# mmbajo/PROBA-V

Measured on AMD Instinct MI355X. Metric: LR-patches/sec fwd+bwd (WDSR-B r12 t9, 16x16, bs128), higher is better.
Workload: dtype f32 (products as 3 scaled-fp16-piece MFMA products, f32 accumulate)

## Files before the change

proba-v_amd/csrc/kernels_direct.hip:

```cpp
#include "probav_common.h"
#include "x6_device.h"

namespace probav {

__device__ __forceinline__ int reflect_idx(int i, int n) {
    i = i < 0 ? -i : i;
    return i >= n ? 2 * n - 2 - i : i;
}

template <int COUT_T, int VEC>
__global__ __launch_bounds__(256) void conv_direct_fwd_kernel(
    ConvGeom g, const float* __restrict__ x, const float* __restrict__ gate, const float* __restrict__ w,
    const float* __restrict__ bias, const float* __restrict__ skip, float* __restrict__ y)
{
    const long nvox = (long)g.N * g.Ho * g.Wo * g.To;
    const long v = (long)blockIdx.x * 256 + threadIdx.x;
    if (v >= nvox) return;
    const int co0 = blockIdx.y * COUT_T;
    long r = v;
    const int t = (int)(r % g.To); r /= g.To;
    const int wo = (int)(r % g.Wo); r /= g.Wo;
    const int h = (int)(r % g.Ho);
    const int n = (int)(r / g.Ho);

// ... 103 lines not shown
#pragma unroll
            for (int dh = 0; dh < 3; ++dh)
#pragma unroll
                for (int dw = 0; dw < 3; ++dw)
#pragma unroll
                    for (int dt = 0; dt < 3; ++dt) {
                        const float xv = ip[(dh * Wp + dw) * Tp + dt];
                        const float4 q = wt[(dh * 3 + dw) * 3 + dt];
                        acc.x = fmaf(xv, q.x, acc.x); acc.y = fmaf(xv, q.y, acc.y); acc.z = fmaf(xv, q.z, acc.z); acc.w = fmaf(xv, q.w, acc.w);
                    }
            if (g.relu) { acc.x = fmaxf(acc.x, 0.f); acc.y = fmaxf(acc.y, 0.f); acc.z = fmaxf(acc.z, 0.f); acc.w = fmaxf(acc.w, 0.f); }
            *reinterpret_cast<float4*>(yrow + (long)v * 32 + 4 * cg) = acc;
            omax = fmaxf(fmaxf(omax, fmaxf(fabsf(acc.x), fabsf(acc.y))), fmaxf(fabsf(acc.z), fabsf(acc.w)));
        }
    }
    if (amax && n_prev >= 0) amax_commit(omax, amax + n_prev);
}

bool conv3d_cin1_forward_supported(const ConvGeom& g)
{
    return g.Cin == 1 && g.Cout == 32 && g.kh == 3 && g.kw == 3 && g.kt == 3 && g.ph == 1 && g.pw == 1 && g.pt == 1 && !g.reflect_hw && !g.reflect_t &&
           g.Ho == g.Hi && g.Wo == g.Wi && g.To == g.Ti && g.To >= 2 && (g.Wi + 2) * (g.Ti + 2) * 3 * sizeof(float) <= 48 * 1024;
}
int conv3d_cin1_forward(const ConvGeom& g, const float* x, const float* w, const float* bias, float* y, unsigned* amax, hipStream_t s)
{
    if (!conv3d_cin1_forward_supported(g)) { set_error("conv3d_cin1_forward: unsupported geometry", hipSuccess); return PROBAV_EINVAL; }
    const long nrows = (long)g.N * g.Ho;
    const size_t lds = (size_t)3 * (g.Wi + 2) * (g.Ti + 2) * sizeof(float);
    hipLaunchKernelGGL(conv3_cin1_fwd_kernel, dim3((unsigned)((nrows + C1_ROWS - 1) / C1_ROWS)), dim3(256), lds, s, g, x, w, bias, y, amax);
    return check_launch("conv3_cin1_fwd");
}

int conv3d_direct_forward(const ConvGeom& g, const float* x, const float* gate, const float* w,
                          const float* bias, const float* skip, float* y, hipStream_t s)
{
    if (g.N <= 0) return PROBAV_OK;
    if (g.Cout % 32 == 0) return launch_fwd<32>(g, x, gate, w, bias, skip, y, s);
    if (g.Cout % 25 == 0) return launch_fwd<25>(g, x, gate, w, bias, skip, y, s);
    if (g.Cout % 9 == 0)  return launch_fwd<9>(g, x, gate, w, bias, skip, y, s);
    if (g.Cout % 4 == 0)  return launch_fwd<4>(g, x, gate, w, bias, skip, y, s);
    return launch_fwd<1>(g, x, gate, w, bias, skip, y, s);
}

bool conv3d_up_forward_supported(const ConvGeom& g)
{
    return g.Cin == 32 && g.Cout == 9 && g.kh == 3 && g.kw == 3 && g.kt == 3 && g.ph == 0 && g.pw == 0 && g.pt == 0 && !g.reflect_hw && !g.reflect_t &&
           g.Ti == 3 && g.To == 1 && g.Ho == g.Hi - 2 && g.Wo == g.Wi - 2 && g.Wo == 16;
}
bool conv3d_up_bwd_data_supported(const ConvGeom& g)
{
    return g.Cin == 9 && g.Cout == 32 && g.kh == 3 && g.kw == 3 && g.kt == 3 && g.ph == 2 && g.pw == 2 && g.pt == 2 && !g.reflect_hw && !g.reflect_t &&
           g.Ti == 1 && g.To == 3 && g.Ho == g.Hi + 2 && g.Wo == g.Wi + 2 && g.Wi <= 30;
}
__global__ __launch_bounds__(256) void conv3_up_fwd_kernel(ConvGeom g, const float* __restrict__ x, const float* __restrict__ w,
                                                          const float* __restrict__ bias, float* __restrict__ y)
{
    extern __shared__ float up_lds[];
    float* sW = up_lds;
    float* sX = sW + 27 * 32 * 9;
    const int tid = threadIdx.x;
    const int rowf = g.Wi * 3 * 32;
    if ((reinterpret_cast<unsigned long>(w) & 15) == 0) {
        for (int i = tid; i < 27 * 32 * 9 / 4; i += 256) reinterpret_cast<float4*>(sW)[i] = reinterpret_cast<const float4*>(w)[i];
    } else {
        for (int i = tid; i < 27 * 32 * 9; i += 256) sW[i] = w[i];
    }
    const int wo = tid >> 4, kp = tid & 15;
    for (int row = blockIdx.x; row < g.N * g.Ho; row += gridDim.x) {
    const int n = row / g.Ho, h = row - n * g.Ho;
    __syncthreads();
    const float4* xr = reinterpret_cast<const float4*>(x + ((long)n * g.Hi + h) * rowf);
    for (int i = tid; i < 3 * rowf / 4; i += 256) reinterpret_cast<float4*>(sX)[i] = xr[i];
    __syncthreads();
    float acc[9];
#pragma unroll
    for (int j = 0; j < 9; ++j) acc[j] = 0.f;
#pragma unroll 2
    for (int q = 0; q < 54; ++q) {
        const int k = kp + 16 * q;
        const int tap = k >> 5, ci = k & 31;
        const int a = tap / 9, bc = tap - 9 * a, b = bc / 3, c = bc - 3 * b;
        const float xv = sX[a * rowf + ((wo + b) * 3 + c) * 32 + ci];
        const float* wr = sW + k * 9;
#pragma unroll
        for (int j = 0; j < 9; ++j) acc[j] = fmaf(xv, wr[j], acc[j]);
    }
#pragma unroll
    for (int j = 0; j < 9; ++j) {
        float v = acc[j];
#pragma unroll
        for (int m = 1; m < 16; m <<= 1) v += __shfl_xor(v, m, 64);
        acc[j] = v;
    }
    if (kp < 9) {
        float o = 0.f;
#pragma unroll
        for (int j = 0; j < 9; ++j) o = kp == j ? acc[j] : o;
        o += bias ? bias[kp] : 0.f;
        if (g.relu) o = fmaxf(o, 0.f);
        y[(((long)n * g.Ho + h) * g.Wo + wo) * 9 + kp] = o;
    }
    }
}
__global__ __launch_bounds__(256) void conv3_up_bwd_data_kernel(ConvGeom g, const float* __restrict__ dy, const float* __restrict__ wT,
                                                               const float* __restrict__ bias, float* __restrict__ dx, unsigned* __restrict__ amax)
{
    extern __shared__ float up_lds[];
    float* sW = up_lds;
    float* sD = sW + 27 * 9 * 32;
    const int tid = threadIdx.x;
    const int Wp = g.Wi + 4;
    if ((reinterpret_cast<unsigned long>(wT) & 15) == 0) {
        for (int i = tid; i < 27 * 9 * 32 / 4; i += 256) reinterpret_cast<float4*>(sW)[i] = reinterpret_cast<const float4*>(wT)[i];
    } else {
        for (int i = tid; i < 27 * 9 * 32; i += 256) sW[i] = wT[i];
    }
    __shared__ float red[4];
    for (int row = blockIdx.x; row < g.N * g.Ho; row += gridDim.x) {
    const int n = row / g.Ho, h = row - n * g.Ho;
    __syncthreads();
    for (int i = tid; i < 3 * Wp * 9; i += 256) {
        const int a = i / (Wp * 9), r = i - a * Wp * 9, wp = r / 9, co = r - 9 * wp;
        const int ih = h + a - 2, iw = wp - 2;
        sD[i] = (ih >= 0 && ih < g.Hi && iw >= 0 && iw < g.Wi) ? dy[(((long)n * g.Hi + ih) * g.Wi + iw) * 9 + co] : 0.f;
    }
    __syncthreads();
    float omax = 0.f;
    const int items = g.Wo * 3 * 8;
    for (int it = tid; it < items; it += 256) {
        const int cg = it & 7, wt = it >> 3, wo = wt / 3, t = wt - 3 * wo;
        float4 acc = bias ? make_float4(bias[4 * cg], bias[4 * cg + 1], bias[4 * cg + 2], bias[4 * cg + 3]) : make_float4(0.f, 0.f, 0.f, 0.f);
#pragma unroll
        for (int a = 0; a < 3; ++a)
#pragma unroll
            for (int b = 0; b < 3; ++b) {
                const float* dp = sD + (a * Wp + wo + b) * 9;
                const float* wp = sW + (((a * 3 + b) * 3 + (2 - t)) * 9) * 32 + 4 * cg;
#pragma unroll
                for (int co = 0; co < 9; ++co) {
                    const float d = dp[co];
                    const float4 q = *reinterpret_cast<const float4*>(wp + co * 32);
                    acc.x = fmaf(d, q.x, acc.x); acc.y = fmaf(d, q.y, acc.y); acc.z = fmaf(d, q.z, acc.z); acc.w = fmaf(d, q.w, acc.w);
                }
            }
        *reinterpret_cast<float4*>(dx + ((((long)n * g.Ho + h) * g.Wo + wo) * 3 + t) * 32 + 4 * cg) = acc;
        omax = fmaxf(fmaxf(omax, fmaxf(fabsf(acc.x), fabsf(acc.y))), fmaxf(fabsf(acc.z), fabsf(acc.w)));
    }
    if (amax) {
#pragma unroll
        for (int o = 32; o; o >>= 1) omax = fmaxf(omax, __shfl_xor(omax, o, 64));
        if ((tid & 63) == 0) red[tid >> 6] = omax;
        __syncthreads();
        if (tid == 0) {
            const float m = fmaxf(fmaxf(red[0], red[1]), fmaxf(red[2], red[3]));
            atomicMax(amax + n, __float_as_uint(m));
        }
    }
    }
}
int conv3d_up_forward(const ConvGeom& g, const float* x, const float* w, const float* bias, float* y, hipStream_t s)
{
    if (!conv3d_up_forward_supported(g)) { set_error("conv3d_up_forward: unsupported geometry", hipSuccess); return PROBAV_EINVAL; }
    const size_t lds = ((size_t)27 * 32 * 9 + (size_t)3 * g.Wi * 3 * 32) * sizeof(float);
    hipLaunchKernelGGL(conv3_up_fwd_kernel, dim3((unsigned)(g.N * g.Ho < 512 ? g.N * g.Ho : 512)), dim3(256), lds, s, g, x, w, bias, y);
    return check_launch("conv3_up_fwd");
}
int conv3d_up_bwd_data(const ConvGeom& g, const float* dy, const float* wT, const float* bias, float* dx, unsigned* amax, hipStream_t s)
{
    if (!conv3d_up_bwd_data_supported(g)) { set_error("conv3d_up_bwd_data: unsupported geometry", hipSuccess); return PROBAV_EINVAL; }
    const size_t lds = ((size_t)27 * 9 * 32 + (size_t)3 * (g.Wi + 4) * 9) * sizeof(float);
    hipLaunchKernelGGL(conv3_up_bwd_data_kernel, dim3((unsigned)(g.N * g.Ho < 768 ? g.N * g.Ho : 768)), dim3(256), lds, s, g, dy, wT, bias, dx, amax);
    return check_launch("conv3_up_bwd_data");
}

template <int KH, int KW, int KT, int CI_PER>
__global__ __launch_bounds__(256) void conv_direct_wgrad_kernel(
    ConvGeom g, const float* __restrict__ x, const float* __restrict__ dy, const float* __restrict__ gate,
    float* __restrict__ partial, float* __restrict__ partial_b, long vox_per_chunk)
{
    constexpr int TAPS = KH * KW * KT;
    const int tid = threadIdx.x;
    const int co = blockIdx.y * 32 + (tid & 31);
    const bool co_ok = co < g.Cout;
    const int ci0 = (blockIdx.z * 8 + (tid >> 5)) * CI_PER;
    const long nvox = (long)g.N * g.Ho * g.Wo * g.To;
    const long v0 = (long)blockIdx.x * vox_per_chunk;
    const long v1 = v0 + vox_per_chunk < nvox ? v0 + vox_per_chunk : nvox;

    float acc[TAPS][CI_PER];
#pragma unroll
    for (int tp = 0; tp < TAPS; ++tp)
#pragma unroll
        for (int k = 0; k < CI_PER; ++k) acc[tp][k] = 0.f;
    float accb = 0.f;
    const bool vec4 = (CI_PER % 4 == 0) && (g.Cin % 4 == 0) && (ci0 + CI_PER <= g.Cin);

    for (long v = v0; v < v1; ++v) {
        long r = v;
        const int t = (int)(r % g.To); r /= g.To;
        const int wo = (int)(r % g.Wo); r /= g.Wo;
        const int h = (int)(r % g.Ho);
        const int n = (int)(r / g.Ho);
        float d = 0.f;
        if (co_ok) {
            d = dy[v * g.Cout + co];
            if (gate) d = gate[v * g.Cout + co] > 0.f ? d : 0.f;
        }
        accb += d;
#pragma unroll
        for (int a = 0; a < KH; ++a) {
            int ih = h + a - g.ph;
            if (g.reflect_hw) ih = reflect_idx(ih, g.Hi);
            else if (ih < 0 || ih >= g.Hi) continue;
#pragma unroll
            for (int b = 0; b < KW; ++b) {
                int iw = wo + b - g.pw;
                if (g.reflect_hw) iw = reflect_idx(iw, g.Wi);
                else if (iw < 0 || iw >= g.Wi) continue;
// ... 415 lines not shown
```

proba-v_amd/csrc/kernels_small.hip:

```cpp
#include "probav_common.h"
#include "../../include/probav_hip.h"
#include <cstdlib>
#include <vector>
#include <functional>
#include <stdio.h>
#include <string.h>

namespace probav {

static thread_local char g_err[512] = "";
void set_error(const char* what, hipError_t e)
{
    if (e != hipSuccess) snprintf(g_err, sizeof(g_err), "%s: %s", what, hipGetErrorString(e));
    else snprintf(g_err, sizeof(g_err), "%s", what);
}
const char* last_error() { return g_err; }
int check_launch(const char* what)
{
    hipError_t e = hipGetLastError();
    if (e != hipSuccess) { set_error(what, e); return PROBAV_EHIP; }
    return PROBAV_OK;
}

__device__ __forceinline__ float wave_sum(float v)
// ... 233 lines not shown
        for (size_t i = (size_t)blockIdx.x * 256 + threadIdx.x; i < n; i += stride) m = fmaxf(m, fabsf(x[i]));
    }
#pragma unroll
    for (int o = 32; o; o >>= 1) m = fmaxf(m, __shfl_xor(m, o, 64));
    __shared__ float wm[4];
    if ((threadIdx.x & 63) == 0) wm[threadIdx.x >> 6] = m;
    __syncthreads();
    if (threadIdx.x == 0) {
        m = fmaxf(fmaxf(wm[0], wm[1]), fmaxf(wm[2], wm[3]));
        atomicMax(slot, __float_as_uint(m));
    }
}
int amax_tensor(const float* x, size_t per_sample, int N, unsigned* slots, hipStream_t s)
{
    if (N < 1) return PROBAV_OK;
    size_t blocks = (per_sample / 4 + 255) / 256;
    if (blocks < 1) blocks = 1;
    const size_t cap = N >= 2048 ? 1 : 2048 / (size_t)N;
    if (blocks > cap) blocks = cap;
    hipLaunchKernelGGL(amax_kernel, dim3((unsigned)blocks, (unsigned)N), dim3(256), 0, s, x, per_sample, slots);
    return check_launch("amax");
}

__global__ __launch_bounds__(256) void amax_columns_kernel(const float* __restrict__ w, long rows, int cols, unsigned* __restrict__ slots)
{
    __shared__ float part[256];
    const int per = 256 / cols, c = threadIdx.x % cols, r0 = threadIdx.x / cols;
    float m = 0.f;
    if (r0 < per) for (long r = r0; r < rows; r += per) m = fmaxf(m, fabsf(w[r * cols + c]));
    part[threadIdx.x] = m;
    __syncthreads();
    if (threadIdx.x < cols) {
        for (int k = 1; k < per; ++k) m = fmaxf(m, part[k * cols + threadIdx.x]);
        slots[threadIdx.x] = __float_as_uint(m);
    }
}
int amax_columns(const float* w, long rows, int cols, unsigned* slots, hipStream_t s)
{
    if (cols < 1 || cols > 256) { set_error("amax_columns: 1 <= cols <= 256", hipSuccess); return PROBAV_EINVAL; }
    hipLaunchKernelGGL(amax_columns_kernel, dim3(1), dim3(256), 0, s, w, rows, cols, slots);
    return check_launch("amax_columns");
}

__global__ __launch_bounds__(64) void wn_backward_kernel(const WnLayer* __restrict__ layers, int nl,
                                                        const float* __restrict__ params, const float* __restrict__ dweff,
                                                        const float* __restrict__ inv_norm, float* __restrict__ grads)
{
    int co;
    const WnLayer L = layers[find_layer(layers, nl, blockIdx.x, co)];
    const float* v = params + L.v_off;
    const float* dw = dweff + L.w_off;
    const int lane = threadIdx.x;
    float dot = 0.f;
    for (int k = lane; k < L.K; k += 64) dot = fmaf(dw[(long)k * L.Cout + co], v[(long)k * L.Cout + co], dot);
    dot = wave_sum(dot);
    const float inv = inv_norm[L.n_off + co];
    const float gg = params[L.g_off + co];
    const bool clamped = inv >= 1e6f;
    const float proj = clamped ? 0.f : dot * inv * inv;
    if (lane == 0) grads[L.g_off + co] = dot * inv;
    for (int k = lane; k < L.K; k += 64) {
        const long i = (long)k * L.Cout + co;
        grads[L.v_off + i] = gg * inv * (dw[i] - v[i] * proj);
    }
}

int wn_forward(const WnLayer* d_layers, int nlayers, int cout_total, int cin_total, const float* params,
               float* weff, float* weffT, float* inv_norm, unsigned* amax, hipStream_t s)
{
    hipLaunchKernelGGL(wn_forward_kernel<false>, dim3(cout_total), dim3(64), 0, s, d_layers, nlayers, const_cast<float*>(params), weff, weffT, inv_norm, amax,
                       (const float*)nullptr, (float*)nullptr, (float*)nullptr, OptCoef());
    int rc = check_launch("wn_forward");
    if (rc || !amax) return rc;
    hipLaunchKernelGGL(wn_rowmax_kernel, dim3(cin_total), dim3(64), 0, s, d_layers, nlayers, weff, amax + 2 * nlayers + cout_total, amax, params);
    return check_launch("wn_rowmax");
}
int optimizer_wn_step(const WnLayer* d_layers, int nlayers, int cout_total, int cin_total, float* params, const float* grad, float* m, float* v,
                      float lr, float b1, float b2, float eps, float c_g, float c_m, float c_v,
                      float* weff, float* weffT, float* inv_norm, unsigned* amax, hipStream_t s)
{
    OptCoef oc = {lr, b1, b2, eps, c_g, c_m, c_v};
    hipLaunchKernelGGL(wn_forward_kernel<true>, dim3(cout_total), dim3(64), 0, s, d_layers, nlayers, params, weff, weffT, inv_norm, amax, grad, m, v, oc);
    int rc = check_launch("optimizer_wn_step");
    if (rc || !amax) return rc;
    hipLaunchKernelGGL(wn_rowmax_kernel, dim3(cin_total), dim3(64), 0, s, d_layers, nlayers, weff, amax + 2 * nlayers + cout_total, amax, params);
    return check_launch("wn_rowmax");
}
int optimizer_wn_step_guarded(const WnLayer* d_layers, int nlayers, int cout_total, int cin_total, float* params, const float* grad, float* m, float* v,
                              float lr, float b1, float b2, float eps, float c_g, float c_m, float c_v,
                              float* weff, float* weffT, float* inv_norm, unsigned* amax, float* ema, float ema_mom, const probav_guard_ctl* ctl, hipStream_t s)
{
    OptCoef oc = {lr, b1, b2, eps, c_g, c_m, c_v};
    hipLaunchKernelGGL(wn_forward_guard_kernel, dim3(cout_total), dim3(64), 0, s, d_layers, nlayers, params, weff, weffT, inv_norm, amax, grad, m, v, oc, ctl, ema, ema_mom);
    int rc = check_launch("optimizer_wn_step_guarded");
    if (rc || !amax) return rc;
    hipLaunchKernelGGL(wn_rowmax_kernel, dim3(cin_total), dim3(64), 0, s, d_layers, nlayers, weff, amax + 2 * nlayers + cout_total, amax, params);
    return check_launch("wn_rowmax");
}
int wn_backward(const WnLayer* d_layers, int nlayers, int cout_total, const float* params,
                const float* dweff, const float* inv_norm, float* grads, hipStream_t s)
{
    hipLaunchKernelGGL(wn_backward_kernel, dim3(cout_total), dim3(64), 0, s, d_layers, nlayers, params, dweff, inv_norm, grads);
    return check_launch("wn_backward");
}

__global__ __launch_bounds__(256) void head_kernel(const float* __restrict__ x, float* __restrict__ xn,
                                                  float* __restrict__ mn, int nhw, int T, int C, float mean, float stdv, unsigned* __restrict__ zero, int nzero)
{
    const int i = blockIdx.x * 256 + threadIdx.x;
    for (int z = i; z < nzero; z += gridDim.x * 256) zero[z] = 0u;
    if (i >= nhw * C) return;
// ... 319 lines not shown

__device__ __forceinline__ int fold_srcs(int i, int n, int p, int (&u)[3])
{
    int c = 0;
    u[c++] = i + p;
    for (int j = 1; j <= p; ++j) {
        if (i == j) u[c++] = p - j;
        if (i == n - 1 - j) u[c++] = n - 1 + p + j;
    }
    return c;
}
__global__ __launch_bounds__(256) void reflect_fold3_kernel(const float* __restrict__ dpad, float* __restrict__ dx, int N, int H, int W,
                                                           int T, int C, int ph, int pw, int pt)
{
    const long i = (long)blockIdx.x * 256 + threadIdx.x;
    if (i >= (long)N * H * W * T * C) return;
    long r = i;
    const int c = (int)(r % C); r /= C;
    const int t = (int)(r % T); r /= T;
    const int w = (int)(r % W); r /= W;
    const int h = (int)(r % H);
    const int n = (int)(r / H);
    int hs[3], ws[3], ts[3];
    const int nh = fold_srcs(h, H, ph, hs), nw = fold_srcs(w, W, pw, ws), nt = fold_srcs(t, T, pt, ts);
    const int Hp = H + 2 * ph, Wp = W + 2 * pw, Tp = T + 2 * pt;
    float s = 0.f;
    for (int a = 0; a < nh; ++a)
        for (int b = 0; b < nw; ++b)
            for (int d = 0; d < nt; ++d)
                s += dpad[((((long)n * Hp + hs[a]) * Wp + ws[b]) * Tp + ts[d]) * C + c];
    dx[i] = s;
}
int reflect_fold3(const float* dpad, float* dx, int N, int H, int W, int T, int C, int ph, int pw, int pt, hipStream_t s)
{
    if (ph < 0 || pw < 0 || pt < 0 || ph > 2 || pw > 2 || pt > 2 || H <= 2 * ph || W <= 2 * pw || T <= 2 * pt) {
        set_error("reflect_fold3: pads must be 0..2 and smaller than half the extent", hipSuccess); return PROBAV_EINVAL;
    }
    const long n = (long)N * H * W * T * C;
    hipLaunchKernelGGL(reflect_fold3_kernel, dim3((unsigned)((n + 255) / 256)), dim3(256), 0, s, dpad, dx, N, H, W, T, C, ph, pw, pt);
    return check_launch("reflect_fold3");
}

__global__ __launch_bounds__(256) void clip_round_kernel(const float* __restrict__ in, float* __restrict__ out, size_t n, float lo, float hi)
{
    const size_t i = (size_t)blockIdx.x * 256 + threadIdx.x;
    if (i < n) out[i] = rintf(fminf(fmaxf(in[i], lo), hi));
}
int clip_round(const float* in, float* out, size_t n, float lo, float hi, hipStream_t s)
{
    hipLaunchKernelGGL(clip_round_kernel, dim3((unsigned)((n + 255) / 256)), dim3(256), 0, s, in, out, n, lo, hi);
    return check_launch("clip_round");
}

__global__ __launch_bounds__(256) void shift_loss_fwd_kernel(
    const float* __restrict__ hr, const uint8_t* __restrict__ mask, const float* __restrict__ pred, int S, int border,
    double* __restrict__ cand)
{
    const int b = blockIdx.x, i = blockIdx.y, lane = threadIdx.x & 63, wave = threadIdx.x >> 6;
    const int L = S - 2 * border, ns = 2 * border + 1, nshift = ns * ns;
    const float* H = hr + (long)b * S * S;
    const uint8_t* M = mask + (long)b * S * S;
    const float* P = pred + (long)b * S * S;
    for (int j = wave; j < ns; j += 4) {
        const int sft = i * ns + j;
        constexpr int U = 4;
        const int n = L * L;
        double cnt = 0.0, dsum = 0.0;
        for (int k0 = lane; k0 < n; k0 += 64 * U) {
            float m[U], h[U], q[U];
#pragma unroll
            for (int u = 0; u < U; ++u) {
                const int k = k0 + 64 * u < n ? k0 + 64 * u : k0;
                const int r = k / L, c = k - r * L;
                m[u] = M[(i + r) * S + j + c] ? 1.f : 0.f;
                h[u] = H[(i + r) * S + j + c];
                q[u] = P[(border + r) * S + border + c];
            }
#pragma unroll
            for (int u = 0; u < U; ++u)
                if (k0 + 64 * u < n) { cnt += (double)m[u]; dsum += (double)(h[u] - q[u] * m[u]); }
        }
        cnt = wave_sum(cnt); dsum = wave_sum(dsum);
        const double bias = dsum / cnt;
        double s1 = 0.0, s2 = 0.0;
        for (int k0 = lane; k0 < n; k0 += 64 * U) {
            float h[U], q[U]; bool mk[U];
#pragma unroll
            for (int u = 0; u < U; ++u) {
                const int k = k0 + 64 * u < n ? k0 + 64 * u : k0;
                const int r = k / L, c = k - r * L;
                mk[u] = M[(i + r) * S + j + c] != 0;
                h[u] = H[(i + r) * S + j + c];
                q[u] = P[(border + r) * S + border + c];
            }
#pragma unroll
            for (int u = 0; u < U; ++u)
                if (k0 + 64 * u < n) {
                    const double m = mk[u] ? 1.0 : 0.0;
                    const double e = (double)h[u] - ((double)q[u] + bias) * m;
                    s1 += fabs(e);
                    s2 += e * e;
                }
        }
        s1 = wave_sum(s1) / cnt; s2 = wave_sum(s2) / cnt;
        if (lane == 0) { cand[((long)b * nshift + sft) * 2] = s1; cand[((long)b * nshift + sft) * 2 + 1] = s2; }
    }
}

__global__ __launch_bounds__(64) void batch_mean_kernel(const float* __restrict__ a, const float* __restrict__ b2,
                                                       float* __restrict__ ma, float* __restrict__ mb, int n)
{
    double s1 = 0.0, s2 = 0.0;
    for (int i = threadIdx.x; i < n; i += 64) { s1 += (double)a[i]; s2 += (double)b2[i]; }
    s1 = wave_sum(s1); s2 = wave_sum(s2);
    if (threadIdx.x == 0) { *ma = (float)(s1 / n); *mb = (float)(s2 / n); }
}

#define SHIFT_NO_CANDIDATE __builtin_nan("")
__global__ __launch_bounds__(1024) void shift_select_mean_kernel(const double* __restrict__ cand, int B, int nshift, float max_val,
                                                                float* __restrict__ l1_out, float* __restrict__ l2_out, float* __restrict__ cpsnr_out,
                                                                int* __restrict__ arg_l1, int* __restrict__ arg_l2, float* __restrict__ ma, float* __restrict__ mb)
{
    __shared__ float sl1[1024], sl2[1024];
    const int b = threadIdx.x;
    if (b < B) {
        const double2* c = reinterpret_cast<const double2*>(cand) + (long)b * nshift;
        double best1 = 1e300, best2 = 1e300;
        int a1 = 0, a2 = 0;
#pragma unroll 7
        for (int sft = 0; sft < nshift; ++sft) {
            const double2 v = c[sft];
            if (v.x < best1) { best1 = v.x; a1 = sft; }
            if (v.y < best2) { best2 = v.y; a2 = sft; }
        }
        if (!(best1 < 1e300)) best1 = SHIFT_NO_CANDIDATE;
        if (!(best2 < 1e300)) best2 = SHIFT_NO_CANDIDATE;
        sl1[b] = l1_out[b] = (float)best1;
        sl2[b] = l2_out[b] = (float)best2;
        cpsnr_out[b] = (float)(10.0 * log10((double)max_val * (double)max_val / best2));
        arg_l1[b] = a1;
        arg_l2[b] = a2;
    }
    __syncthreads();
    if (threadIdx.x < 64) {
        double s1 = 0.0, s2 = 0.0;
        for (int i = threadIdx.x; i < B; i += 64) { s1 += (double)sl1[i]; s2 += (double)sl2[i]; }
        s1 = wave_sum(s1); s2 = wave_sum(s2);
        if (threadIdx.x == 0) { *ma = (float)(s1 / B); *mb = (float)(s2 / B); }
    }
}

__global__ __launch_bounds__(64) void shift_select_kernel(const double* __restrict__ cand, int B, int nshift, float max_val,
                                                         float* __restrict__ l1_out, float* __restrict__ l2_out, float* __restrict__ cpsnr_out,
                                                         int* __restrict__ arg_l1, int* __restrict__ arg_l2)
{
    const int b = blockIdx.x * 64 + threadIdx.x;
    if (b >= B) return;
    const double2* c = reinterpret_cast<const double2*>(cand) + (long)b * nshift;
    double best1 = 1e300, best2 = 1e300;
    int a1 = 0, a2 = 0;
#pragma unroll 7
    for (int sft = 0; sft < nshift; ++sft) {
        const double2 v = c[sft];
        if (v.x < best1) { best1 = v.x; a1 = sft; }
        if (v.y < best2) { best2 = v.y; a2 = sft; }
    }
    if (!(best1 < 1e300)) best1 = SHIFT_NO_CANDIDATE;
    if (!(best2 < 1e300)) best2 = SHIFT_NO_CANDIDATE;
    l1_out[b] = (float)best1;
    l2_out[b] = (float)best2;
    cpsnr_out[b] = (float)(10.0 * log10((double)max_val * (double)max_val / best2));
    arg_l1[b] = a1;
    arg_l2[b] = a2;
}

int shift_loss_forward(const float* hr, const uint8_t* mask, const float* pred, int B, int S, int border,
                       float* l1, float* l2, float* cpsnr, int* arg_l1, int* arg_l2, float* mean_l1, float* mean_l2,
                       float max_val, hipStream_t s)
{
    if (B <= 0 || border < 0 || S <= 2 * border) { set_error("shift_loss_forward: bad shape (size must exceed 2 * border)", hipSuccess); return PROBAV_EINVAL; }
    const int ns = 2 * border + 1;
    static double* cand = nullptr;
    static size_t cand_n = 0;
    const size_t need = (size_t)B * ns * ns * 2;
    if (need > cand_n) {
        if (cand) (void)hipFree(cand);
        cand = nullptr; cand_n = 0;
        hipError_t err = hipMalloc((void**)&cand, need * sizeof(double));
        if (err != hipSuccess) { set_error("shift_loss_forward: scratch allocation", err); return PROBAV_EHIP; }
        cand_n = need;
    }
    hipLaunchKernelGGL(shift_loss_fwd_kernel, dim3(B, ns), dim3(256), 0, s, hr, mask, pred, S, border, cand);
    if (B <= 1024) {
        hipLaunchKernelGGL(shift_select_mean_kernel, dim3(1), dim3((unsigned)((B + 63) / 64 * 64)), 0, s, cand, B, ns * ns, max_val, l1, l2, cpsnr, arg_l1, arg_l2, mean_l1, mean_l2);
        return check_launch("shift_loss_forward");
    }
    hipLaunchKernelGGL(shift_select_kernel, dim3((unsigned)((B + 63) / 64)), dim3(64), 0, s, cand, B, ns * ns, max_val, l1, l2, cpsnr, arg_l1, arg_l2);
    hipLaunchKernelGGL(batch_mean_kernel, dim3(1), dim3(64), 0, s, l1, l2, mean_l1, mean_l2, B);
    return check_launch("shift_loss_forward");
}

__global__ __launch_bounds__(256) void shift_loss_bwd_kernel(
    const float* __restrict__ hr, const uint8_t* __restrict__ mask, const float* __restrict__ pred,
    const int* __restrict__ arg, int S, int border, int which, const float* __restrict__ upstream, float inv_b,
    float* __restrict__ dpred)
{
    const float scale = (upstream ? upstream[0] : 1.f) * inv_b;
    const int b = blockIdx.x, tid = threadIdx.x, lane = tid & 63, wave = tid >> 6;
    const int L = S - 2 * border, ns = 2 * border + 1;
    const float* H = hr + (long)b * S * S;
    const uint8_t* M = mask + (long)b * S * S;
    const float* P = pred + (long)b * S * S;
    float* G = dpred + (long)b * S * S;
    const int sft = arg[b], i = sft / ns, j = sft - i * ns;
    __shared__ double red[2][4];
    double cnt = 0.0, dsum = 0.0;
    for (int k = tid; k < L * L; k += 256) {
        const int r = k / L, c = k - r * L;
        const float m = M[(i + r) * S + j + c] ? 1.f : 0.f;
        cnt += (double)m;
        dsum += (double)(H[(i + r) * S + j + c] - P[(border + r) * S + border + c] * m);
    }
    cnt = wave_sum(cnt); dsum = wave_sum(dsum);
    if (lane == 0) { red[0][wave] = cnt; red[1][wave] = dsum; }
    __syncthreads();
    cnt = red[0][0] + red[0][1] + red[0][2] + red[0][3];
    dsum = red[1][0] + red[1][1] + red[1][2] + red[1][3];
    const double bias = dsum / cnt;
    __syncthreads();
    double ssum = 0.0;
    for (int k = tid; k < L * L; k += 256) {
        const int r = k / L, c = k - r * L;
        const double m = M[(i + r) * S + j + c] ? 1.0 : 0.0;
        const double e = (double)H[(i + r) * S + j + c] - ((double)P[(border + r) * S + border + c] + bias) * m;
        const double sg = which == 1 ? (e > 0.0 ? 1.0 : (e < 0.0 ? -1.0 : 0.0)) : 2.0 * e;
        ssum += sg * m;
    }
    ssum = wave_sum(ssum);
    if (lane == 0) red[0][wave] = ssum;
    __syncthreads();
    ssum = red[0][0] + red[0][1] + red[0][2] + red[0][3];
    for (int k = tid; k < S * S; k += 256) {
        const int Y = k / S, X = k - Y * S, r = Y - border, c = X - border;
        float gk = 0.f;
        if (r >= 0 && r < L && c >= 0 && c < L) {
            const double m = M[(i + r) * S + j + c] ? 1.0 : 0.0;
            const double e = (double)H[(i + r) * S + j + c] - ((double)P[Y * S + X] + bias) * m;
            const double sg = which == 1 ? (e > 0.0 ? 1.0 : (e < 0.0 ? -1.0 : 0.0)) : 2.0 * e;
            gk = (float)(-(m / cnt) * (sg - ssum / cnt) * (double)scale);
        }
        G[k] = gk;
    }
}
int shift_loss_backward(const float* hr, const uint8_t* mask, const float* pred, const int* arg, int B, int S,
                        int border, int which, const float* upstream, float* dpred, hipStream_t s)
{
    if (which != 1 && which != 2) { set_error("shift_loss_backward: which must be 1 (L1) or 2 (L2)", hipSuccess); return PROBAV_EINVAL; }
    if (B <= 0 || border < 0 || S <= 2 * border) { set_error("shift_loss_backward: bad shape (size must exceed 2 * border)", hipSuccess); return PROBAV_EINVAL; }
    hipLaunchKernelGGL(shift_loss_bwd_kernel, dim3(B), dim3(256), 0, s, hr, mask, pred, arg, S, border, which, upstream, 1.0f / (float)B, dpred);
    return check_launch("shift_loss_backward");
}

__device__ __forceinline__ int mirror(int i, int n) { return i < 0 ? -i : (i >= n ? 2 * n - 2 - i : i); }

__device__ __forceinline__ double block_sum(double v, double* red, int tid)
{
    v = wave_sum(v);
    __syncthreads();
    if ((tid & 63) == 0) red[tid >> 6] = v;
    __syncthreads();
    return red[0] + red[1] + red[2] + red[3];
}

__global__ __launch_bounds__(256) void shift_l1edge_fwd_kernel(
    const float* __restrict__ hr, const uint8_t* __restrict__ mask, const float* __restrict__ pred, int S, int border, float pi,
    float* __restrict__ loss_out, int* __restrict__ arg_out)
{
    extern __shared__ float sD[];
    __shared__ double red[4];
    const int b = blockIdx.x, tid = threadIdx.x;
    const int L = S - 2 * border, ns = 2 * border + 1, nshift = ns * ns;
    const float* H = hr + (long)b * S * S;
    const uint8_t* M = mask + (long)b * S * S;
    const float* P = pred + (long)b * S * S;
    double best = 1e300;
    int abest = 0;
    for (int sft = 0; sft < nshift; ++sft) {
        const int i = sft / ns, j = sft - i * ns;
        double cnt = 0.0, dsum = 0.0;
        for (int k = tid; k < L * L; k += 256) {
            const int r = k / L, c = k - r * L;
            const float m = M[(i + r) * S + j + c] ? 1.f : 0.f;
            cnt += (double)m;
            dsum += (double)(H[(i + r) * S + j + c] - P[(border + r) * S + border + c] * m);
        }
        cnt = block_sum(cnt, red, tid);
        dsum = block_sum(dsum, red, tid);
        const double bias = dsum / cnt;
        double s1 = 0.0;
        for (int k = tid; k < L * L; k += 256) {
            const int r = k / L, c = k - r * L;
            const double m = M[(i + r) * S + j + c] ? 1.0 : 0.0;
            const double e = (double)H[(i + r) * S + j + c] - ((double)P[(border + r) * S + border + c] + bias) * m;
            sD[k] = (float)e;
// ... 492 lines not shown
```

Baseline: 20920.

## Tile up-conv forward over rows, register-cache loss and weight-norm loads

The upsampling conv forward now gives each block four output rows, one wave per row, with a padded LDS layout. Each lane computes four output pixels so weight reads from LDS are reused, and the input and weight loads are batched into registers before being written to LDS. The shift-loss forward kernel now runs one wave per shift candidate across more blocks and keeps the patch and its mask bits in registers. The shift-loss backward and weight-norm gradient kernels are also changed to load their data once into registers instead of re-reading it in a second pass. This adds register pressure and hardcodes the 18-pixel input width.

Measured after the change: 20820. About the same (-0.5%).

```diff
diff --git a/proba-v_amd/csrc/kernels_direct.hip b/proba-v_amd/csrc/kernels_direct.hip
--- a/proba-v_amd/csrc/kernels_direct.hip
+++ b/proba-v_amd/csrc/kernels_direct.hip
@@ -179,54 +179,98 @@
     return g.Cin == 9 && g.Cout == 32 && g.kh == 3 && g.kw == 3 && g.kt == 3 && g.ph == 2 && g.pw == 2 && g.pt == 2 && !g.reflect_hw && !g.reflect_t &&
            g.Ti == 1 && g.To == 3 && g.Ho == g.Hi + 2 && g.Wo == g.Wi + 2 && g.Wi <= 30;
 }
+constexpr int UP_ROWS = 4;
+constexpr int UP_WI = 18;
+constexpr int UP_PIX = 3 * 32 + 16;
 __global__ __launch_bounds__(256) void conv3_up_fwd_kernel(ConvGeom g, const float* __restrict__ x, const float* __restrict__ w,
                                                           const float* __restrict__ bias, float* __restrict__ y)
 {
     extern __shared__ float up_lds[];
     float* sW = up_lds;
     float* sX = sW + 27 * 32 * 9;
-    const int tid = threadIdx.x;
-    const int rowf = g.Wi * 3 * 32;
+    const int tid = threadIdx.x, lane = tid & 63, wave = tid >> 6;
+    const int groups = (g.Ho + UP_ROWS - 1) / UP_ROWS;
+    const int n = blockIdx.x / groups, h0 = (blockIdx.x - n * groups) * UP_ROWS;
+    float* spare = sX + 96;
+    const int nrows = (g.Ho - h0 < UP_ROWS ? g.Ho - h0 : UP_ROWS) + 2;
+    const float4* xr = reinterpret_cast<const float4*>(x + ((long)n * g.Hi + h0) * UP_WI * 96);
+    constexpr int XQ = ((UP_ROWS + 2) * UP_WI * 24 + 255) / 256;
+    float4 tx[XQ];
+#pragma unroll
+    for (int j = 0; j < XQ; ++j) { const int i = tid + 256 * j; tx[j] = xr[i < nrows * UP_WI * 24 ? i : 0]; }
+    static_assert(XQ == 11, "the two groups below");
+#define UP_KEEP4(t) "+v"(t.x), "+v"(t.y), "+v"(t.z), "+v"(t.w)
+    asm volatile("" : UP_KEEP4(tx[0]), UP_KEEP4(tx[1]), UP_KEEP4(tx[2]), UP_KEEP4(tx[3]), UP_KEEP4(tx[4]), UP_KEEP4(tx[5]));
+    asm volatile("" : UP_KEEP4(tx[6]), UP_KEEP4(tx[7]), UP_KEEP4(tx[8]), UP_KEEP4(tx[9]), UP_KEEP4(tx[10]));
+#undef UP_KEEP4
+#pragma unroll
+    for (int j = 0; j < XQ; ++j) {
+        const int i = tid + 256 * j;
+        const int px = i / 24, v = i - 24 * px;
+        *reinterpret_cast<float4*>(i < nrows * UP_WI * 24 ? sX + px * UP_PIX + 4 * v : spare) = tx[j];
+    }
     if ((reinterpret_cast<unsigned long>(w) & 15) == 0) {
-        for (int i = tid; i < 27 * 32 * 9 / 4; i += 256) reinterpret_cast<float4*>(sW)[i] = reinterpret_cast<const float4*>(w)[i];
+        constexpr int WQ = (27 * 32 * 9 / 4 + 255) / 256;
+        float4 tw[WQ];
+#pragma unroll
+        for (int j = 0; j < WQ; ++j) { const int i = tid + 256 * j; tw[j] = reinterpret_cast<const float4*>(w)[i < 27 * 32 * 9 / 4 ? i : 0]; }
+#pragma unroll
+        for (int j = 0; j < WQ; ++j) { const int i = tid + 256 * j; *reinterpret_cast<float4*>(i < 27 * 32 * 9 / 4 ? sW + 4 * i : spare) = tw[j]; }
     } else {
-        for (int i = tid; i < 27 * 32 * 9; i += 256) sW[i] = w[i];
-    }
-    const int wo = tid >> 4, kp = tid & 15;
-    for (int row = blockIdx.x; row < g.N * g.Ho; row += gridDim.x) {
-    const int n = row / g.Ho, h = row - n * g.Ho;
-    __syncthreads();
-    const float4* xr = reinterpret_cast<const float4*>(x + ((long)n * g.Hi + h) * rowf);
-    for (int i = tid; i < 3 * rowf / 4; i += 256) reinterpret_cast<float4*>(sX)[i] = xr[i];
-    __syncthreads();
-    float acc[9];
-#pragma unroll
-    for (int j = 0; j < 9; ++j) acc[j] = 0.f;
-#pragma unroll 2
+        constexpr int WQ = (27 * 32 * 9 + 255) / 256;
+        float tw[WQ];
+#pragma unroll
+        for (int j = 0; j < WQ; ++j) { const int i = tid + 256 * j; tw[j] = w[i < 27 * 32 * 9 ? i : 0]; }
+#pragma unroll
+        for (int j = 0; j < WQ; ++j) { const int i = tid + 256 * j; *(i < 27 * 32 * 9 ? sW + i : spare) = tw[j]; }
+    }
+    __syncthreads();
+    const int h = h0 + wave;
+    if (h >= g.Ho) return;
+    const int kp = lane & 15, cgp = lane >> 4;
+    float acc[4][9];
+#pragma unroll
+    for (int i = 0; i < 4; ++i)
+#pragma unroll
+        for (int j = 0; j < 9; ++j) acc[i][j] = 0.f;
+    const float* xb = sX + (wave * UP_WI + cgp) * UP_PIX + kp;
+    const float* wb = sW + kp * 9;
+#pragma unroll
     for (int q = 0; q < 54; ++q) {
-        const int k = kp + 16 * q;
-        const int tap = k >> 5, ci = k & 31;
+        const int tap = q >> 1;
         const int a = tap / 9, bc = tap - 9 * a, b = bc / 3, c = bc - 3 * b;
-        const float xv = sX[a * rowf + ((wo + b) * 3 + c) * 32 + ci];
-        const float* wr = sW + k * 9;
-#pragma unroll
-        for (int j = 0; j < 9; ++j) acc[j] = fmaf(xv, wr[j], acc[j]);
-    }
-#pragma unroll
-    for (int j = 0; j < 9; ++j) {
-        float v = acc[j];
-#pragma unroll
-        for (int m = 1; m < 16; m <<= 1) v += __shfl_xor(v, m, 64);
-        acc[j] = v;
-    }
+        const float* xp = xb + (a * UP_WI + b) * UP_PIX + c * 32 + 16 * (q & 1);
+        const float* wr = wb + 16 * q * 9;
+        float wv[9];
+#pragma unroll
+        for (int j = 0; j < 9; ++j) wv[j] = wr[j];
+#pragma unroll
+        for (int i = 0; i < 4; ++i) {
+            const float xv = xp[4 * i * UP_PIX];
+#pragma unroll
+            for (int j = 0; j < 9; ++j) acc[i][j] = fmaf(xv, wv[j], acc[i][j]);
+        }
+    }
+#pragma unroll
+    for (int i = 0; i < 4; ++i)
+#pragma unroll
+        for (int j = 0; j < 9; ++j) {
+            float v = acc[i][j];
+#pragma unroll
+            for (int m = 1; m < 16; m <<= 1) v += __shfl_xor(v, m, 64);
+            acc[i][j] = v;
+        }
     if (kp < 9) {
-        float o = 0.f;
-#pragma unroll
-        for (int j = 0; j < 9; ++j) o = kp == j ? acc[j] : o;
-        o += bias ? bias[kp] : 0.f;
-        if (g.relu) o = fmaxf(o, 0.f);
-        y[(((long)n * g.Ho + h) * g.Wo + wo) * 9 + kp] = o;
-    }
+        const float bv = bias ? bias[kp] : 0.f;
+#pragma unroll
+        for (int i = 0; i < 4; ++i) {
+            float o = 0.f;
+#pragma unroll
+            for (int j = 0; j < 9; ++j) o = kp == j ? acc[i][j] : o;
+            o += bv;
+            if (g.relu) o = fmaxf(o, 0.f);
+            y[(((long)n * g.Ho + h) * g.Wo + cgp + 4 * i) * 9 + kp] = o;
+        }
     }
 }
 __global__ __launch_bounds__(256) void conv3_up_bwd_data_kernel(ConvGeom g, const float* __restrict__ dy, const float* __restrict__ wT,
@@ -288,9 +332,8 @@
 int conv3d_up_forward(const ConvGeom& g, const float* x, const float* w, const float* bias, float* y, hipStream_t s)
 {
     if (!conv3d_up_forward_supported(g)) { set_error("conv3d_up_forward: unsupported geometry", hipSuccess); return PROBAV_EINVAL; }
-    const size_t lds = ((size_t)27 * 32 * 9 + (size_t)3 * g.Wi * 3 * 32) * sizeof(float);
-    hipLaunchKernelGGL(conv3_up_fwd_kernel, dim3((unsigned)(g.N * g.Ho < 512 ? g.N * g.Ho : 512)), dim3(256), lds, s, g, x, w, bias, y);
-    return check_launch("conv3_up_fwd");
+    const size_t lds = ((size_t)27 * 32 * 9 + (size_t)(UP_ROWS + 2) * UP_WI * UP_PIX) * sizeof(float);
+    return launch_lds<conv3_up_fwd_kernel>("conv3_up_fwd", dim3((unsigned)(g.N * ((g.Ho + UP_ROWS - 1) / UP_ROWS))), dim3(256), lds, s, g, x, w, bias, y);
 }
 int conv3d_up_bwd_data(const ConvGeom& g, const float* dy, const float* wT, const float* bias, float* dx, unsigned* amax, hipStream_t s)
 {
diff --git a/proba-v_amd/csrc/kernels_small.hip b/proba-v_amd/csrc/kernels_small.hip
--- a/proba-v_amd/csrc/kernels_small.hip
+++ b/proba-v_amd/csrc/kernels_small.hip
@@ -309,11 +309,33 @@
     const float* dw = dweff + L.w_off;
     const int lane = threadIdx.x;
     float dot = 0.f;
-    for (int k = lane; k < L.K; k += 64) dot = fmaf(dw[(long)k * L.Cout + co], v[(long)k * L.Cout + co], dot);
-    dot = wave_sum(dot);
     const float inv = inv_norm[L.n_off + co];
     const float gg = params[L.g_off + co];
     const bool clamped = inv >= 1e6f;
+    constexpr int WN_Q = 14;
+    if (L.K <= WN_Q * 64) {
+        float qd[WN_Q], qv[WN_Q];
+#pragma unroll
+        for (int j = 0; j < WN_Q; ++j) {
+            const int k = lane + 64 * j;
+            const long i = (long)(k < L.K ? k : 0) * L.Cout + co;
+            const float a = dw[i], b = v[i];
+            qd[j] = k < L.K ? a : 0.f; qv[j] = k < L.K ? b : 0.f;
+        }
+#pragma unroll
+        for (int j = 0; j < WN_Q; ++j) dot = fmaf(qd[j], qv[j], dot);
+        dot = wave_sum(dot);
+        const float proj = clamped ? 0.f : dot * inv * inv;
+        if (lane == 0) grads[L.g_off + co] = dot * inv;
+#pragma unroll
+        for (int j = 0; j < WN_Q; ++j) {
+            const int k = lane + 64 * j;
+            if (k < L.K) grads[L.v_off + (long)k * L.Cout + co] = gg * inv * (qd[j] - qv[j] * proj);
+        }
+        return;
+    }
+    for (int k = lane; k < L.K; k += 64) dot = fmaf(dw[(long)k * L.Cout + co], v[(long)k * L.Cout + co], dot);
+    dot = wave_sum(dot);
     const float proj = clamped ? 0.f : dot * inv * inv;
     if (lane == 0) grads[L.g_off + co] = dot * inv;
     for (int k = lane; k < L.K; k += 64) {
@@ -739,29 +761,67 @@
     return check_launch("clip_round");
 }
 
-__global__ __launch_bounds__(256) void shift_loss_fwd_kernel(
+constexpr int SHIFT_FWD_WAVES = 8;
+constexpr int SHIFT_FWD_Q = 28;
+__global__ __launch_bounds__(64 * SHIFT_FWD_WAVES) void shift_loss_fwd_kernel(
     const float* __restrict__ hr, const uint8_t* __restrict__ mask, const float* __restrict__ pred, int S, int border,
     double* __restrict__ cand)
 {
-    const int b = blockIdx.x, i = blockIdx.y, lane = threadIdx.x & 63, wave = threadIdx.x >> 6;
+    const int b = blockIdx.x, i = blockIdx.y, lane = threadIdx.x & 63;
+    const int wave = __builtin_amdgcn_readfirstlane((int)(threadIdx.x >> 6));
     const int L = S - 2 * border, ns = 2 * border + 1, nshift = ns * ns;
-    const float* H = hr + (long)b * S * S;
-    const uint8_t* M = mask + (long)b * S * S;
-    const float* P = pred + (long)b * S * S;
-    for (int j = wave; j < ns; j += 4) {
-        const int sft = i * ns + j;
+    const int j = blockIdx.z * SHIFT_FWD_WAVES + wave;
+    if (j >= ns) return;
+    const int sft = i * ns + j, n = L * L;
+    const float* H = hr + (long)b * S * S + i * S + j;
+    const uint8_t* M = mask + (long)b * S * S + i * S + j;
+    const float* P = pred + (long)b * S * S + border * S + border;
+    double cnt = 0.0, dsum = 0.0, s1 = 0.0, s2 = 0.0;
+    if (n <= 64 * SHIFT_FWD_Q) {
+        static_assert(SHIFT_FWD_Q <= 32, "the mask of a lane's pixels is one 32-bit word");
+        const int dr = 64 / L, dc = 64 - dr * L;
+        float h[SHIFT_FWD_Q], q[SHIFT_FWD_Q];
+        unsigned clear = 0u;
+        int r = lane / L, c = lane - r * L;
+#pragma unroll
+        for (int u = 0; u < SHIFT_FWD_Q; ++u) {
+            const bool in = lane + 64 * u < n;
+            const unsigned o = in ? (unsigned)(r * S + c) : 0u;
+            const uint8_t mu = *(M + o);
+            const float hu = *reinterpret_cast<const float*>(reinterpret_cast<const char*>(H) + 4u * o);
+            const float qu = *reinterpret_cast<const float*>(reinterpret_cast<const char*>(P) + 4u * o);
+            clear |= (in && mu ? 1u : 0u) << u;
+            h[u] = in ? hu : 0.f;
+            q[u] = in ? qu : 0.f;
+            c += dc; r += dr;
+            if (c >= L) { c -= L; ++r; }
+        }
+        cnt = (double)__popc(clear);
+#pragma unroll
+        for (int u = 0; u < SHIFT_FWD_Q; ++u) {
+            const float m = (clear >> u) & 1u ? 1.f : 0.f;
+            dsum += (double)(h[u] - q[u] * m);
+        }
+        cnt = wave_sum(cnt); dsum = wave_sum(dsum);
+        const double bias = dsum / cnt;
+#pragma unroll
+        for (int u = 0; u < SHIFT_FWD_Q; ++u) {
+            const double m = (clear >> u) & 1u ? 1.0 : 0.0;
+            const double e = (double)h[u] - ((double)q[u] + bias) * m;
+            s1 += fabs(e);
+            s2 += e * e;
+        }
+    } else {
         constexpr int U = 4;
-        const int n = L * L;
-        double cnt = 0.0, dsum = 0.0;
         for (int k0 = lane; k0 < n; k0 += 64 * U) {
             float m[U], h[U], q[U];
 #pragma unroll
             for (int u = 0; u < U; ++u) {
                 const int k = k0 + 64 * u < n ? k0 + 64 * u : k0;
                 const int r = k / L, c = k - r * L;
-                m[u] = M[(i + r) * S + j + c] ? 1.f : 0.f;
-                h[u] = H[(i + r) * S + j + c];
-                q[u] = P[(border + r) * S + border + c];
+                m[u] = M[r * S + c] ? 1.f : 0.f;
+                h[u] = H[r * S + c];
+                q[u] = P[r * S + c];
             }
 #pragma unroll
             for (int u = 0; u < U; ++u)
@@ -769,16 +829,15 @@
         }
         cnt = wave_sum(cnt); dsum = wave_sum(dsum);
         const double bias = dsum / cnt;
-        double s1 = 0.0, s2 = 0.0;
         for (int k0 = lane; k0 < n; k0 += 64 * U) {
             float h[U], q[U]; bool mk[U];
 #pragma unroll
             for (int u = 0; u < U; ++u) {
                 const int k = k0 + 64 * u < n ? k0 + 64 * u : k0;
                 const int r = k / L, c = k - r * L;
-                mk[u] = M[(i + r) * S + j + c] != 0;
-                h[u] = H[(i + r) * S + j + c];
-                q[u] = P[(border + r) * S + border + c];
+                mk[u] = M[r * S + c] != 0;
+                h[u] = H[r * S + c];
+                q[u] = P[r * S + c];
             }
 #pragma unroll
             for (int u = 0; u < U; ++u)
@@ -789,9 +848,9 @@
                     s2 += e * e;
                 }
         }
-        s1 = wave_sum(s1) / cnt; s2 = wave_sum(s2) / cnt;
-        if (lane == 0) { cand[((long)b * nshift + sft) * 2] = s1; cand[((long)b * nshift + sft) * 2 + 1] = s2; }
-    }
+    }
+    s1 = wave_sum(s1) / cnt; s2 = wave_sum(s2) / cnt;
+    if (lane == 0) { cand[((long)b * nshift + sft) * 2] = s1; cand[((long)b * nshift + sft) * 2 + 1] = s2; }
 }
 
 __global__ __launch_bounds__(64) void batch_mean_kernel(const float* __restrict__ a, const float* __restrict__ b2,
@@ -877,7 +936,7 @@
         if (err != hipSuccess) { set_error("shift_loss_forward: scratch allocation", err); return PROBAV_EHIP; }
         cand_n = need;
     }
-    hipLaunchKernelGGL(shift_loss_fwd_kernel, dim3(B, ns), dim3(256), 0, s, hr, mask, pred, S, border, cand);
+    hipLaunchKernelGGL(shift_loss_fwd_kernel, dim3(B, ns, (ns + SHIFT_FWD_WAVES - 1) / SHIFT_FWD_WAVES), dim3(64 * (ns < SHIFT_FWD_WAVES ? ns : SHIFT_FWD_WAVES)), 0, s, hr, mask, pred, S, border, cand);
     if (B <= 1024) {
         hipLaunchKernelGGL(shift_select_mean_kernel, dim3(1), dim3((unsigned)((B + 63) / 64 * 64)), 0, s, cand, B, ns * ns, max_val, l1, l2, cpsnr, arg_l1, arg_l2, mean_l1, mean_l2);
         return check_launch("shift_loss_forward");
@@ -887,6 +946,7 @@
     return check_launch("shift_loss_forward");
 }
 
+constexpr int SHIFT_BWD_Q = 7;
 __global__ __launch_bounds__(256) void shift_loss_bwd_kernel(
     const float* __restrict__ hr, const uint8_t* __restrict__ mask, const float* __restrict__ pred,
     const int* __restrict__ arg, int S, int border, int which, const float* __restrict__ upstream, float inv_b,
@@ -901,42 +961,79 @@
     float* G = dpred + (long)b * S * S;
     const int sft = arg[b], i = sft / ns, j = sft - i * ns;
     __shared__ double red[2][4];
-    double cnt = 0.0, dsum = 0.0;
-    for (int k = tid; k < L * L; k += 256) {
-        const int r = k / L, c = k - r * L;
-        const float m = M[(i + r) * S + j + c] ? 1.f : 0.f;
-        cnt += (double)m;
-        dsum += (double)(H[(i + r) * S + j + c] - P[(border + r) * S + border + c] * m);
-    }
-    cnt = wave_sum(cnt); dsum = wave_sum(dsum);
-    if (lane == 0) { red[0][wave] = cnt; red[1][wave] = dsum; }
-    __syncthreads();
-    cnt = red[0][0] + red[0][1] + red[0][2] + red[0][3];
-    dsum = red[1][0] + red[1][1] + red[1][2] + red[1][3];
-    const double bias = dsum / cnt;
-    __syncthreads();
-    double ssum = 0.0;
-    for (int k = tid; k < L * L; k += 256) {
-        const int r = k / L, c = k - r * L;
-        const double m = M[(i + r) * S + j + c] ? 1.0 : 0.0;
-        const double e = (double)H[(i + r) * S + j + c] - ((double)P[(border + r) * S + border + c] + bias) * m;
-        const double sg = which == 1 ? (e > 0.0 ? 1.0 : (e < 0.0 ? -1.0 : 0.0)) : 2.0 * e;
-        ssum += sg * m;
+    double cnt = 0.0, dsum = 0.0, bias, ssum = 0.0;
+    const int n = L * L;
+    if (n <= 256 * SHIFT_BWD_Q) {
+        float h[SHIFT_BWD_Q], q[SHIFT_BWD_Q];
+        unsigned clear = 0u;
+#pragma unroll
+        for (int u = 0; u < SHIFT_BWD_Q; ++u) {
+            const int k = tid + 256 * u;
+            const bool in = k < n;
+            const int r = k / L, c = k - r * L;
+            const int o = in ? r * S + c : 0;
+            const uint8_t mu = M[i * S + j + o];
+            const float hu = H[i * S + j + o], qu = P[border * S + border + o];
+            clear |= (in && mu ? 1u : 0u) << u;
+            h[u] = in ? hu : 0.f;
+            q[u] = in ? qu : 0.f;
+        }
+        cnt = (double)__popc(clear);
+#pragma unroll
+        for (int u = 0; u < SHIFT_BWD_Q; ++u) {
+            const float m = (clear >> u) & 1u ? 1.f : 0.f;
+            dsum += (double)(h[u] - q[u] * m);
+        }
+        cnt = wave_sum(cnt); dsum = wave_sum(dsum);
+        if (lane == 0) { red[0][wave] = cnt; red[1][wave] = dsum; }
+        __syncthreads();
+        cnt = red[0][0] + red[0][1] + red[0][2] + red[0][3];
+        dsum = red[1][0] + red[1][1] + red[1][2] + red[1][3];
+        bias = dsum / cnt;
+        __syncthreads();
+#pragma unroll
+        for (int u = 0; u < SHIFT_BWD_Q; ++u) {
+            const double m = (clear >> u) & 1u ? 1.0 : 0.0;
+            const double e = (double)h[u] - ((double)q[u] + bias) * m;
+            const double sg = which == 1 ? (e > 0.0 ? 1.0 : (e < 0.0 ? -1.0 : 0.0)) : 2.0 * e;
+            ssum += sg * m;
+        }
+    } else {
+        for (int k = tid; k < n; k += 256) {
+            const int r = k / L, c = k - r * L;
+            const float m = M[(i + r) * S + j + c] ? 1.f : 0.f;
+            cnt += (double)m;
+            dsum += (double)(H[(i + r) * S + j + c] - P[(border + r) * S + border + c] * m);
+        }
+        cnt = wave_sum(cnt); dsum = wave_sum(dsum);
+        if (lane == 0) { red[0][wave] = cnt; red[1][wave] = dsum; }
+        __syncthreads();
+        cnt = red[0][0] + red[0][1] + red[0][2] + red[0][3];
+        dsum = red[1][0] + red[1][1] + red[1][2] + red[1][3];
+        bias = dsum / cnt;
+        __syncthreads();
+        for (int k = tid; k < n; k += 256) {
+            const int r = k / L, c = k - r * L;
+            const double m = M[(i + r) * S + j + c] ? 1.0 : 0.0;
+            const double e = (double)H[(i + r) * S + j + c] - ((double)P[(border + r) * S + border + c] + bias) * m;
+            const double sg = which == 1 ? (e > 0.0 ? 1.0 : (e < 0.0 ? -1.0 : 0.0)) : 2.0 * e;
+            ssum += sg * m;
+        }
     }
     ssum = wave_sum(ssum);
     if (lane == 0) red[0][wave] = ssum;
     __syncthreads();
     ssum = red[0][0] + red[0][1] + red[0][2] + red[0][3];
+#pragma unroll 4
     for (int k = tid; k < S * S; k += 256) {
         const int Y = k / S, X = k - Y * S, r = Y - border, c = X - border;
-        float gk = 0.f;
-        if (r >= 0 && r < L && c >= 0 && c < L) {
-            const double m = M[(i + r) * S + j + c] ? 1.0 : 0.0;
-            const double e = (double)H[(i + r) * S + j + c] - ((double)P[Y * S + X] + bias) * m;
-            const double sg = which == 1 ? (e > 0.0 ? 1.0 : (e < 0.0 ? -1.0 : 0.0)) : 2.0 * e;
-            gk = (float)(-(m / cnt) * (sg - ssum / cnt) * (double)scale);
-        }
-        G[k] = gk;
+        const bool in = r >= 0 && r < L && c >= 0 && c < L;
+        const int o = in ? r * S + c : 0;
+        const double m = M[i * S + j + o] ? 1.0 : 0.0;
+        const double e = (double)H[i * S + j + o] - ((double)P[border * S + border + o] + bias) * m;
+        const double sg = which == 1 ? (e > 0.0 ? 1.0 : (e < 0.0 ? -1.0 : 0.0)) : 2.0 * e;
+        const float gk = (float)(-(m / cnt) * (sg - ssum / cnt) * (double)scale);
+        G[k] = in ? gk : 0.f;
     }
 }
 int shift_loss_backward(const float* hr, const uint8_t* mask, const float* pred, const int* arg, int B, int S,
```
